# edwardyang12/Dex-NERF

Measured on AMD Instinct MI355X. Metric: rays/sec (64+128 samples) + PSNR vs ref, 400x400 scene, higher is better.
Workload: dtype bf16; 1 GPU; C2 render: 400x400 rays/step/GPU, 64 coarse + 128 fine samples, coarse+fine FlexibleNeRFModel D8/W256/skip4 + viewdirs, PE L=10/4, 20 Dex thresholds, validation mode (det. resampling, no noise)

## Files before the change

dex-nerf_amd/csrc/api.cpp:

```cpp
#include <cmath>
#include <cstdlib>
#include <cstring>
#include <utility>
#include <vector>

#include "../../include/dexnerf_hip_ext.h"
#include "../../include/dexnerf_hip_normals.h"
#include "../../include/dexnerf_hip_quantile.h"
#include "dn_common.h"
#include "composite_body.h"
#include "dn_rng.h"
#include "mlp_layout.h"

namespace dn {

static thread_local char g_err[512] = "";

void set_error(const char* fmt, ...) {
  va_list ap;
  va_start(ap, fmt);
  vsnprintf(g_err, sizeof(g_err), fmt, ap);
  va_end(ap);
}

// ... 18 lines not shown
    int cus = 256;
    if (hipDeviceGetAttribute(&cus, hipDeviceAttributeMultiprocessorCount, dev) != hipSuccess || cus <= 0) cus = 256;
    cache[dev] = cus;
  }
  return cache[dev];
}

static size_t align256(size_t v) { return (v + 255) & ~static_cast<size_t>(255); }

struct Workspace {
  float *z_c, *rf_c, *w_c, *z_f, *rf_f, *g_rf;
  unsigned* absmax_part;
  unsigned* status;
  size_t bytes;
};

static Workspace carve(void* base, int64_t n, int nc, int nf, bool train = false) {
  Workspace w{};
  size_t off = 0;
  auto take = [&](size_t floats) {
    float* p = base ? reinterpret_cast<float*>(static_cast<char*>(base) + off) : nullptr;
    off += align256(floats * sizeof(float));
    return p;
  };
  w.z_c = take(static_cast<size_t>(n) * nc);
  w.rf_c = take(static_cast<size_t>(n) * nc * 4);
  w.w_c = take(static_cast<size_t>(n) * nc);
  if (nf > 0) {
    w.z_f = take(static_cast<size_t>(n) * (nc + nf));
    w.rf_f = take(static_cast<size_t>(n) * (nc + nf) * 4);
// ... 85 lines not shown
  if ((rc = dn_coarse_depths(rays, ray_stride, n_rays, num_coarse, lindisp, t_rand, w.z_c, stream))) return rc;
  const bool fine = num_fine > 0;
  DN_REQUIRE(n_thres >= 0 && n_thres <= kMaxThres, "dn_render_rays: at most %d Dex thresholds", kMaxThres);
  auto comp_for = [&](float* rgb, float* acc, float* weights, float* depth, float* dex, int k) {
    CompParams c{};
    c.rgb = rgb; c.acc = acc; c.weights = weights; c.depth = depth; c.dex = dex; c.disp = nullptr;
    c.nonfinite = w.status; c.n_rays = n_rays; c.n_thres = k; c.white = white_background;
    for (int i = 0; i < kMaxThres; ++i) c.th.m[i] = (i < k) ? h_m_thres[i] : 0.0f;
    return c;
  };
  const bool may_fuse = !(noise_std > 0.0f);
  int done = 0;
  {
    const CompParams c = comp_for(rgb_c, acc_c, w.w_c, depth_c, fine ? nullptr : dex_f, fine ? 0 : n_thres);
    if ((rc = run_network_flagged(desc_coarse, precision, packed_coarse, nullptr, nullptr, rays, ray_stride, w.z_c, n_rays,
                                  num_coarse, w.rf_c, w.status + 1, stream, (may_fuse && rgb_c) ? &c : nullptr, &done)))
      return rc;
  }
  if (!done && (rc = volume_render_counting(w.rf_c, w.z_c, rays + 3, ray_stride, noise_c, noise_std, white_background, h_m_thres,
                                            fine ? 0 : n_thres, n_rays, num_coarse, rgb_c, nullptr, acc_c, w.w_c, depth_c,
                                            fine ? nullptr : dex_f, w.status, stream)))
    return rc;
  if (!fine) return 0;
  if ((rc = dn_fine_depths(w.z_c, w.w_c, u, n_rays, num_coarse, num_fine, w.z_f, nullptr, stream))) return rc;
  {
    const CompParams c = comp_for(rgb_f, acc_f, nullptr, depth_f, dex_f, n_thres);
    if ((rc = run_network_flagged(desc_fine, precision, packed_fine, nullptr, nullptr, rays, ray_stride, w.z_f, n_rays,
                                  num_coarse + num_fine, w.rf_f, w.status + 1, stream, (may_fuse && rgb_f) ? &c : nullptr, &done)))
      return rc;
  }
  if (done) return 0;
  return volume_render_counting(w.rf_f, w.z_f, rays + 3, ray_stride, noise_f, noise_std, white_background, h_m_thres, n_thres,
                                n_rays, num_coarse + num_fine, rgb_f, nullptr, acc_f, nullptr, depth_f, dex_f, w.status, stream);
}

extern "C" size_t dn_render_depth_workspace_bytes(int64_t n_rays, int num_coarse, int num_fine) {
  if (n_rays < 0 || num_coarse < 1 || num_fine < 0) return 0;
  return carve_depth(nullptr, n_rays, num_coarse, num_fine).bytes;
}

static int render_rays_depth_impl(const char* who, const dn_mlp_desc* desc_coarse, const void* packed_coarse, const dn_mlp_desc* desc_fine,
                                  const void* packed_fine, int precision, const float* rays, int ray_stride, int64_t n_rays,
                                  int num_coarse, int num_fine, int lindisp, float noise_std, const float* d_m_thres, int n_thres,
// ... 488 lines not shown
```

dex-nerf_amd/csrc/dn_common.h:

```cpp
#pragma once
#include <hip/hip_runtime.h>
#include <cstdarg>
#include <cstdint>
#include <cstdio>

#include "../../include/dexnerf_hip.h"

namespace dn {

constexpr int kWave = 64;

void set_error(const char* fmt, ...);

inline hipStream_t as_stream(dn_stream_t s) { return reinterpret_cast<hipStream_t>(s); }

inline int check_launch(const char* what) {
  hipError_t e = hipGetLastError();
  if (e != hipSuccess) {
    set_error("%s: %s", what, hipGetErrorString(e));
    return -static_cast<int>(e);
  }
  return 0;
}

// ... 18 lines not shown
                                int n_samples, float* depth, float* acc, float* dex, float* qdepth, unsigned* nonfinite,
                                dn_stream_t stream);

int composite_normals_counting(const float* rf, const float* z, const float* rd, int rd_stride, const float* noise, float noise_std,
                               const float* g_pts, const float* d_m_thres, int n_thres, int64_t n_rays, int n_samples, float* depth,
                               float* acc, float* dex, float* normal, float* dex_normal, unsigned* nonfinite, dn_stream_t stream);
int density_seed(float* g_out, int64_t n_points, dn_stream_t stream);
int input_grad_check(const dn_mlp_desc* desc, int precision, const char* who);
int input_grad_points_from_rays(const dn_mlp_desc* desc, int precision, const void* packed_ig, const void* grads, const float* rays,
                                int ray_stride, const float* z_vals, int64_t n_rays, int samples_per_ray, float* d_pts, dn_stream_t stream);

bool weight_grad_pair_fits(const dn_mlp_desc& d);
struct CompParams;
int run_network_flagged(const dn_mlp_desc* desc, int precision, const void* packed, const float* pts, const float* viewdirs,
                        const float* rays, int ray_stride, const float* z_vals, int64_t n_rays, int samples_per_ray, float* out,
                        unsigned* range_flag, dn_stream_t stream, const CompParams* comp = nullptr, int* composited = nullptr);

int coarse_depths_rng(const float* rays, int ray_stride, int64_t n_rays, int num_coarse, int lindisp, const float* t_rand,
                      float* z_vals, const uint32_t* rng_state, dn_stream_t stream);
int fine_depths_rng(const float* z_coarse, const float* weights, const float* u, int64_t n_rays, int num_coarse, int num_fine,
                    float* z_fine, float* z_samples, const uint32_t* rng_state, dn_stream_t stream);
int volume_render_backward_rng(const char* name, const float* rf, const float* z, const float* rd, int rd_stride, const float* noise,
                               float noise_std, int white_background, int64_t n_rays, int n_samples, const float* g_rgb,
                               const float* g_depth, const float* g_acc, const float* g_disp, const float* g_weights, float* g_rf,
                               float* g_z, float* g_rd, const uint32_t* rng_state, uint32_t rng_stream, unsigned* absmax_part,
                               dn_stream_t stream);
int coarse_depths_backward_rng(const float* rays, int ray_stride, int64_t n_rays, int num_coarse, int lindisp, const float* t_rand,
                               const float* g_z, const float* g_z_b, const float* g_z_c, float* g_near_far, const uint32_t* rng_state,
                               dn_stream_t stream);
int fine_depths_backward_sum(const float* z_coarse, const float* z_samples, const float* g_z_fine, const float* g_z_fine_b, int64_t n_rays,
                             int num_coarse, int num_fine, float* g_z_coarse, dn_stream_t stream);
// ... 123 lines not shown
```

dex-nerf_amd/csrc/mlp_fused.hip:

```cpp
#include "mlp_fused_kernel.h"
#include "mlp_internal.h"
#include "mlp_geo48.h"

namespace dn {

DN_FWD32_INSTANCES(DN_FWD32_EXTERN)


template <int BF16, int DENS = 0>
__global__ void pack_kernel(NetLayout L, PackPtrs ptrs, char* __restrict__ packed) {
  using P = Prec<BF16>;
  const int n_bias = L.total_bias_tiles * 32;
  float* bias_out = reinterpret_cast<float*>(packed);
  for (int idx = blockIdx.x * blockDim.x + threadIdx.x; idx < L.bias_bytes / 4; idx += gridDim.x * blockDim.x) {
    float v = 0.0f;
    if (idx < n_bias) {
      const int tile = idx / 32, hh = (idx % 32) / 16, r = idx % 16, s = pack_stage_of_bias_tile(L, tile);
      int src;
      const int n = pack_src_row<32>(L.st[s], tile - L.st[s].bias0, acc_row(r, hh), DENS && s == L.n_stages - 1, &src);
      if (n >= 0) v = ptrs.b[src][n];
    }
    bias_out[idx] = v;
  }
  char* wout = packed + L.bias_bytes;
// ... 51 lines not shown

template <int W, int LX, int LD, int BF16, int PT, int SAVE>
static int launch_forward(FwdParams p, hipStream_t stream) {
  auto kern = mlp_forward_kernel<W, LX, LD, BF16, PT, SAVE>;
  constexpr int WAVES = waves_of<BF16, PT>();
  constexpr int PTS_PER_WG = WAVES * 32 * PT;
  constexpr int KXP = kXyzPanel / (2 * Prec<BF16>::EPP);
  p.n_tiles = (p.n_points + PTS_PER_WG - 1) / PTS_PER_WG;
  constexpr int KDP = round_up(3 + 6 * LD, 16) / (2 * Prec<BF16>::EPP);
  const size_t lds = kRingBytes + p.bias_bytes + WAVES * (kInRows * 32 * PT * sizeof(float) + PT * (KXP + KDP) * kPieceBytes);
  if (int rc = ensure_big_lds(reinterpret_cast<const void*>(kern))) return rc;
  hipLaunchKernelGGL(kern, dim3(static_cast<unsigned>(persistent_grid(p.n_tiles))), dim3(WAVES * 64), lds, stream, p);
  return check_launch("mlp_forward");
}

int dispatch_forward(const dn_mlp_desc& d, int precision, FwdParams& p, hipStream_t stream, const CompParams* comp, int* composited) {
  const bool bf = precision == DN_PREC_BF16;
  const bool hf = precision == DN_PREC_F16;
  const char* region48 = p.packed + core_stream_bytes(p.bias_bytes, p.total_pieces);
  if ((bf || hf) && !read_switches().geom32 && p.act == nullptr && p.mode != 2 && p.n_points < (1LL << 31) - 1024 && g48_supported(d, precision))
    return launch_forward48(d, precision, p, region48, stream, comp, composited);
  if (p.act != nullptr && hf) { set_error("mlp_forward(train): fp16 is a render-only mode"); return DN_E_UNSUPPORTED; }
  if (p.act != nullptr && p.save8) {
    if (!bf || p.mode == 2 || !g48_train_supported(d) || p.n_points >= (1LL << 31) - 1024) {
      set_error("mlp_forward(train, 8-bit saved tensors): bf16 arithmetic, rays / points input, W in {128, 256}, L_xyz in {6, 10}, a depth the 48-point kernel holds in LDS");
      return DN_E_UNSUPPORTED;
    }
    return launch_forward48(d, precision, p, region48, stream);
  }
  const int prec_arg = bf ? 1 : hf ? 2 : 0;
  const int save = p.act != nullptr ? 1 : 0;
#define DN_CASE(W_, LX_, F_, SAVE_)                                                            \
  if (d.hidden_size == W_ && d.num_encoding_fn_xyz == LX_ && prec_arg == F_ && save == SAVE_) \
    return launch_forward<W_, LX_, 4, F_, 1, SAVE_>(p, stream);
  DN_FWD32_INSTANCES(DN_CASE)
#undef DN_CASE
// ... 108 lines not shown
  if (rc == 0 && g48_supported(d, precision))
    rc = launch_pack48(d, precision, ptrs, static_cast<char*>(packed) + core_stream_bytes(L.bias_bytes, L.total_pieces), as_stream(stream), true);
  return rc;
}

extern "C" int dn_run_network(const dn_mlp_desc* desc, int precision, const void* packed, const float* pts,
                              const float* viewdirs, const float* rays, int ray_stride, const float* z_vals,
                              int64_t n_rays, int samples_per_ray, float* out, dn_stream_t stream) {
  return dn::run_network_flagged(desc, precision, packed, pts, viewdirs, rays, ray_stride, z_vals, n_rays, samples_per_ray, out,
                                 nullptr, stream);
}

int dn::run_network_flagged(const dn_mlp_desc* desc, int precision, const void* packed, const float* pts,
                            const float* viewdirs, const float* rays, int ray_stride, const float* z_vals,
                            int64_t n_rays, int samples_per_ray, float* out, unsigned* range_flag, dn_stream_t stream,
                            const CompParams* comp, int* composited) {
  if (composited) *composited = 0;
  FwdParams p;
  int rc = setup_params(desc, precision, packed, &p);
  if (rc) return rc;
  if (n_rays == 0) return 0;
  DN_REQUIRE(packed && out && n_rays >= 0 && samples_per_ray >= 1, "dn_run_network: bad arguments");
  DN_REQUIRE((reinterpret_cast<uintptr_t>(out) & 15) == 0, "dn_run_network: out must be 16-byte aligned");
  if ((rc = set_point_inputs("dn_run_network", *desc, pts, viewdirs, rays, ray_stride, z_vals, n_rays, samples_per_ray, &p))) return rc;
  p.out = out;
  p.range_flag = range_flag;
  if (p.n_points == 0) return 0;
  return dispatch_forward(*desc, precision, p, as_stream(stream), comp, composited);
}

extern "C" int dn_mlp_forward_encoded(const dn_mlp_desc* desc, int precision, const void* packed, const float* x,
                                      int64_t n_rows, float* out, dn_stream_t stream) {
  FwdParams p;
  int rc = setup_params(desc, precision, packed, &p);
  if (rc) return rc;
  if (n_rows == 0) return 0;
  DN_REQUIRE(packed && x && out && n_rows >= 0, "dn_mlp_forward_encoded: bad arguments");
  DN_REQUIRE((reinterpret_cast<uintptr_t>(out) & 15) == 0, "dn_mlp_forward_encoded: out must be 16-byte aligned");
  p.mode = 2; p.enc = x;
  p.enc_ld = (3 + 6 * desc->num_encoding_fn_xyz) + (desc->use_viewdirs ? 3 + 6 * desc->num_encoding_fn_dir : 0);
  p.n_points = n_rows; p.S = 1; p.out = out;
  if (n_rows == 0) return 0;
  return dispatch_forward(*desc, precision, p, as_stream(stream));
// ... 2 lines not shown
```

dex-nerf_amd/csrc/mlp_fused48.hip:

```cpp
#include "mlp_fused48_kernel.h"

namespace dn {

DN_FWD48_INSTANCES(DN_FWD48_EXTERN)
template <int W, int F, int DC, unsigned MASKC, int VIEWC, int SAVE, int OVLP, int COMP>
__global__ __launch_bounds__(kG48Waves * 64, 2) void mlp_forward_density48_kernel(FwdParams p, G48Params q);
#define DN_FWD48_DENSITY_EXTERN(W, F, DC, MASKC, VIEWC, SAVE, OVLP, COMP) \
  extern template __global__ void mlp_forward_density48_kernel<W, F, DC, MASKC, VIEWC, SAVE, OVLP, COMP>(FwdParams, G48Params);
DN_FWD48_DENSITY(DN_FWD48_DENSITY_EXTERN)

template <int F, int DENS = 0>
__device__ __forceinline__ void pack48_body(const NetLayout& L, const PackPtrs& ptrs, const G48Tables& tabs, char* __restrict__ region);

template <int F, int DENS = 0>
__global__ void pack48_kernel(NetLayout L, PackPtrs ptrs, G48Tables tabs, char* __restrict__ region) {
  pack48_body<F, DENS>(L, ptrs, tabs, region);
}

template <int F>
__global__ void pack48_pair_kernel(NetLayout L, PackPtrs ptrs_a, PackPtrs ptrs_b, G48Tables tabs, char* __restrict__ region_a,
                                   char* __restrict__ region_b) {
  if (blockIdx.y == 0) pack48_body<F>(L, ptrs_a, tabs, region_a);
  else pack48_body<F>(L, ptrs_b, tabs, region_b);
}
// ... 74 lines not shown
  const G48Tables tabs = g48_tables(d);
  const dim3 blocks(pack48_blocks(L), b ? 2 : 1);
  if (b) {
    static_assert(sizeof(NetLayout) + 2 * sizeof(PackPtrs) + sizeof(G48Tables) + 16 <= 4096, "kernel arguments of the pair pack");
    hipLaunchKernelGGL(pack48_pair_kernel<1>, blocks, dim3(256), 0, stream, L, a, *b, tabs, region_a, region_b);
    return check_launch("mlp_pack48_pair");
  }
  with_prec<false>(precision, [&](auto f) {
    constexpr int F = decltype(f)::value;
    auto kern = density ? pack48_kernel<F, 1> : pack48_kernel<F, 0>;
    hipLaunchKernelGGL(kern, blocks, dim3(256), 0, stream, L, a, tabs, region_a);
  });
  return check_launch(density ? "mlp_pack48_density" : "mlp_pack48");
}

int launch_forward48(const dn_mlp_desc& d, int precision, const FwdParams& p_in, const char* region, hipStream_t stream,
                     const CompParams* comp, int* composited) {
  if (composited) *composited = 0;
  NetLayout L;
  build_layout48(d, &L);
  FwdParams p = p_in;
  G48Params q{};
  q.base = region; q.bias_bytes = L.bias_bytes; q.total_pieces = L.total_pieces;
  size_t lds = g48_lds_bytes(L);
  if (lds > 160 * 1024) { set_error("mlp_forward48: %zu bytes of LDS", lds); return DN_E_UNSUPPORTED; }
  const int cus = device_cus();
  const G48Pick pick = g48_pick(d, precision, p, comp, cus, read_switches());
  if (pick.refusal) { set_error("%s", pick.refusal); return DN_E_UNSUPPORTED; }
  const G48Key& k = pick.key;
  const int tile_points = k.SAVE == 3 ? 256 : kG48PointsPerWg;
  p.n_tiles = (p.n_points + tile_points - 1) / tile_points;
  if (k.OVLP == 1) lds += static_cast<size_t>(kG48Waves) * 3 * kG48PointsPerWave * sizeof(float);
  if (k.COMP) {
    q.comp = *comp;
    if (composited) *composited = 1;
  }
  auto launch = [&](auto kern) -> int {
    if (int rc = ensure_big_lds(reinterpret_cast<const void*>(kern))) return rc;
    hipLaunchKernelGGL(kern, dim3(static_cast<unsigned>(persistent_grid(p.n_tiles, cus))), dim3(kG48Waves * 64), lds, stream, p, q);
    return check_launch("mlp_forward48");
  };
#define DN_CASE(KERNEL, W, F, DC, MASKC, VIEWC, SAVE, OVLP, COMP) \
  if (k == G48Key{W, F, DC, MASKC, VIEWC, SAVE, OVLP, COMP}) return launch(KERNEL<W, F, DC, MASKC, VIEWC, SAVE, OVLP, COMP>);
#define DN_CASE_FWD(...) DN_CASE(mlp_forward48_kernel, __VA_ARGS__)
#define DN_CASE_DENSITY(...) DN_CASE(mlp_forward_density48_kernel, __VA_ARGS__)
  if (pick.density) { DN_FWD48_DENSITY(DN_CASE_DENSITY) }
  else { DN_FWD48_INSTANCES(DN_CASE_FWD) }
#undef DN_CASE_DENSITY
#undef DN_CASE_FWD
#undef DN_CASE
  set_error("mlp_forward48: the picked instance is not in the list");
  return DN_E_UNSUPPORTED;
}
// ... 3 lines not shown
```

dex-nerf_amd/csrc/mlp_fused48_kernel.h:

```cpp
#pragma once
#include "mlp_stage48.h"

namespace dn {


template <bool MAY_BE_IDENTITY = true>
__device__ __forceinline__ float pe_value(float xc, f32x4 entry) {
  const float rev = __builtin_amdgcn_fractf(xc * entry[0]) + entry[1];
  const float s = __builtin_amdgcn_sinf(rev);
  if constexpr (MAY_BE_IDENTITY) return entry[2] * xc + entry[3] * s;
  else return s;
}

__device__ __forceinline__ void rotate3(const float (&x)[3], int g, float (&xr)[3]) {
  const unsigned r = static_cast<unsigned>(g) % 3u;
  const unsigned m1 = 0u - (r & 1u), m2 = 0u - (r >> 1);
  const unsigned b0 = __float_as_uint(x[0]), b1 = __float_as_uint(x[1]), b2 = __float_as_uint(x[2]);
  xr[0] = __uint_as_float(b0 ^ ((b0 ^ b1) & m1) ^ ((b0 ^ b2) & m2));
  xr[1] = __uint_as_float(b1 ^ ((b1 ^ b2) & m1) ^ ((b1 ^ b0) & m2));
  xr[2] = __uint_as_float(b2 ^ ((b2 ^ b0) & m1) ^ ((b2 ^ b1) & m2));
}

template <int W, int F, int DC = 0, unsigned MASKC = 0, int VIEWC = 0, int SAVE = 0, int OVLP = 0, int COMP = 0>
__global__ __launch_bounds__(kG48Waves * 64, 2) void mlp_forward48_kernel(FwdParams p, G48Params q) {
// ... 59 lines not shown
      for (int c = 0; c < 3; ++c) dma(p.pts + static_cast<long long>(pt) * 3 + c, c);
      if (p.use_viewdirs) {
        const float* v = p.viewdirs + static_cast<long long>(pt / p.S) * 3;
#pragma unroll
        for (int c = 0; c < 3; ++c) dma(v + c, 7 + 3 * vset + c);
      }
    }
  };

  {
    const f32x4* gsrc = reinterpret_cast<const f32x4*>(q.base);
    f32x4* l = reinterpret_cast<f32x4*>(bias_lds);
    for (int i = threadIdx.x; i < (q.bias_bytes + kG48TableBytes) / 16; i += WAVES * 64) l[i] = gsrc[i];
  }
  issue_inputs(blockIdx.x, 0);
  const unsigned inbuf_addr = static_cast<unsigned>(reinterpret_cast<uintptr_t>((__attribute__((address_space(3))) char*)inbuf));
  auto issue_inputs_flat = [&](int tile, int set) {
    const int ln = fresh_lane();
    int pt = tile * PPG + wave * PPW + ln;
    pt = pt < n_points ? pt : n_points - 1;
    const float* r = p.rays + static_cast<long long>(pt / p.S) * p.ray_stride;
#pragma unroll
    for (int c = 0; c < 6; ++c) dma4_lanes48(r + c, inbuf_addr + c * (PPW * 4));
    dma4_lanes48(p.z + pt, inbuf_addr + 6 * (PPW * 4));
#pragma unroll
    for (int c = 0; c < 3; ++c) dma4_lanes48(r + 8 + c, inbuf_addr + (7 + c) * (PPW * 4) + set * (3 * PPW * 4));
  };

  Pipe48<WAVES> pipe;
  pipe.ring = ring;
// ... 34 lines not shown
    const f32x4* tabx = reinterpret_cast<const f32x4*>(tab_lds) + (lane >> 4) * 16;
#pragma unroll
    for (int u = 0; u < 16; ++u) {
      const f32x4 e = tabx[u];
      tfreq[u] = e[0]; tphase[u] = e[1];
      if (u < 3) { tw_id[u] = e[2]; tw_sin[u] = e[3]; }
    }
  }
  unsigned long long idm[3] = {0ull, 0ull, 0ull};
  if constexpr (OVX) {
    const f32x4* tabx = reinterpret_cast<const f32x4*>(tab_lds) + (lane >> 4) * 16;
#pragma unroll
    for (int u = 0; u < 3; ++u) idm[u] = __ballot(tabx[u][2] != 0.0f);
  }
  const int n_tiles = static_cast<int>(p.n_tiles);
  auto tile_loop = [&](auto role_c) __attribute__((always_inline)) {
  constexpr int ROLE = decltype(role_c)::value;
  if constexpr (SPLIT) first_reads();
  for (int tile = blockIdx.x; tile < n_tiles; tile += gridDim.x, vset = (VSETS == 2 ? vset ^ 1 : (vset == 2 ? 0 : vset + 1))) {
    const char* act_grp[PT] = {};
    const char* mask_base = nullptr;
    if constexpr (SAVE != 0) {
      const long long wt = static_cast<long long>(tile) * WAVES + wave;
#pragma unroll
      for (int t = 0; t < PT; ++t) {
        const long long G = wt * PT + t;
        act_grp[t] = uniform_ptr(p.act + ((G >> 1) * p.act_pieces * 2 + (G & 1)) * kPieceBytes);
      }
      mask_base = uniform_ptr(p.masks + wt * p.mask_words * (2 * kPieceBytes));
    }
    const bool first_tile = tile == static_cast<int>(blockIdx.x);
    if ((!OVL && !OVX) || first_tile) {
      const int ln = fresh_lane();
      const int j = ln & 15;
      const f32x4* tabx = reinterpret_cast<const f32x4*>(tab_lds) + (ln >> 4) * 16;
      char* pex = pex_of(ln);
      if (wave >= 4) asm volatile("s_waitcnt vmcnt(0)" ::: "memory");
      float in[PT][7];
#pragma unroll
      for (int t = 0; t < PT; ++t)
#pragma unroll
        for (int c = 0; c < 7; ++c) in[t][c] = inbuf[c * PPW + t * 16 + j];
      asm volatile("s_waitcnt lgkmcnt(0)" ::: "memory");
      {
        const int nxt = tile + gridDim.x;
        if (nxt < n_tiles) issue_inputs(nxt, vset ^ 1);
      }
#pragma unroll
      for (int t = 0; t < PT; ++t) {
        float x[3];
#pragma unroll
        for (int c = 0; c < 3; ++c)
          x[c] = (p.mode == 0) ? in[t][c] + in[t][3 + c] * in[t][6] : in[t][c];
        float xr[3];
        rotate3(x, ln >> 4, xr);
        BP8 pk[KXP];
#pragma unroll
        for (int k = 0; k < KXP; ++k) {
          BP8 piece;
#pragma unroll
// ... 146 lines not shown
        static_assert(SPLIT, "in-stage encoding: an instance whose pass is compiled per role");
        if constexpr (ROLE == kXsConsumer) asm volatile("s_waitcnt vmcnt(0)" ::: "memory");
        else asm volatile("" ::: "memory");
        const int ln = fresh_lane();
        const int j = ln & 15;
#pragma unroll
        for (int t = 0; t < PT; ++t)
#pragma unroll
          for (int c = 0; c < 7; ++c) in_n[t][c] = inbuf[c * PPW + t * 16 + j];
        tab_addr_v = pipe.ring_addr + kRingBytes + static_cast<unsigned>(q.bias_bytes) + static_cast<unsigned>(ln >> 4) * 256u;
        stash_addr_v = pipe.ring_addr + kRingBytes + static_cast<unsigned>(q.bias_bytes) + kG48TableBytes + wave * (PT * KXP * kPieceBytes) + static_cast<unsigned>(ln) * 16u;
        asm volatile("ds_read_b64 %0, %1" : "=v"(tbl[0]) : "v"(tab_addr_v));
      }
#pragma unroll
      for (int t = 0; t < PT; ++t) ped[t] = *reinterpret_cast<const BP8*>(pex_of(pipe.lane16 >> 4) + t * kPieceBytes);
      asm volatile("s_waitcnt lgkmcnt(0)" : "+v"(ped[0]), "+v"(ped[1]), "+v"(ped[2]), "+v"(pipe.af[0]), "+v"(pipe.af[1]), "+v"(pipe.bias_nxt), "+v"(tbl[0]));
      if constexpr (OVX) {
        const int t2 = tile + 2 * static_cast<int>(gridDim.x);
        issue_inputs_flat(t2 < n_tiles ? t2 : tile, vset);
        const int ln = fresh_lane();
#pragma unroll
        for (int t = 0; t < PT; ++t) {
          float x[3];
#pragma unroll
          for (int c = 0; c < 3; ++c) x[c] = in_n[t][c] + in_n[t][3 + c] * in_n[t][6];
          rotate3(x, ln >> 4, xr_n[t]);
        }
      }
      auto enc_hook = [&](auto b_c, auto w_c) {
        if constexpr (OVX) {
          constexpr int b = decltype(b_c)::value, w = decltype(w_c)::value;
          constexpr int q0 = enc_begin(b, KT_D), cap = enc_cap(b, KT_D);
          auto one = [&](auto q_c) {
            constexpr int qq = decltype(q_c)::value;
// ... 237 lines not shown
      for (; i + 1 < p.D - 1; i += 2) {
        trunk_layer(i, ba, bb);
        trunk_layer(i + 1, bb, ba);
      }
      if (i < p.D - 1) {
        trunk_layer(i, ba, bb);
#pragma unroll
        for (int t = 0; t < PT; ++t)
#pragma unroll
          for (int k = 0; k < KH; ++k) ba[t][k] = bb[t][k];
      }
      if (p.use_viewdirs) heads(ba, bb, std::true_type{});
      else heads(ba, bb, std::false_type{});
    }
    }
    const int lo = fresh_lane();
    if constexpr (COMP != 0) {
      f32x4* stage = reinterpret_cast<f32x4*>(smem + kRingBytes + q.bias_bytes + kG48TableBytes);
#pragma unroll
      for (int t = 0; t < PT; ++t) {
        if (lo < 16) {
          f32x4 o;
          o[0] = out4[t][0]; o[1] = out4[t][1]; o[2] = out4[t][2]; o[3] = out4[t][3];
          stage[wave * PPW + t * 16 + lo] = o;
        }
      }
      asm volatile("s_waitcnt lgkmcnt(0)" ::: "memory");
      __builtin_amdgcn_s_barrier();
      const int S = p.S;
      const int rays_per_tile = PPG / S;
// ... 9 lines not shown
      asm volatile("s_waitcnt lgkmcnt(0)" ::: "memory");
      __builtin_amdgcn_s_barrier();
    } else {
#pragma unroll
      for (int t = 0; t < PT; ++t) {
        const int pt = tile * PPG + wave * PPW + t * 16 + (lo & 15);
        if (pt < n_points && lo < 16) {
          f32x4 o;
          o[0] = out4[t][0]; o[1] = out4[t][1]; o[2] = out4[t][2]; o[3] = out4[t][3];
          __builtin_nontemporal_store(o, reinterpret_cast<f32x4*>(p.out + static_cast<long long>(pt) * 4));
        }
      }
    }
  }
  };
  if constexpr (SPLIT) {
    if (wave < 4) tile_loop(std::integral_constant<int, kXsFetcher>{});
    else tile_loop(std::integral_constant<int, kXsConsumer>{});
  } else {
    tile_loop(std::integral_constant<int, kXsFetcher>{});
  }
  asm volatile("s_waitcnt vmcnt(0) lgkmcnt(0)" ::: "memory");
  if constexpr (F == 2) {
    const bool out_of_range = (trk & 0xFFFFu) >= 0x7C00u || (trk >> 16) >= 0x7C00u;
    if (p.range_flag != nullptr && __ballot(out_of_range) != 0ull && (threadIdx.x & 63) == 0) atomicAdd(p.range_flag, 1u);
  }
}

#define DN_FWD48_PAPER_BF16_ENC(X) X(256, 1, 8, 0x10u, 1, 0, 2, 0)
#define DN_FWD48_PAPER_BF16_PLAIN(X) X(256, 1, 8, 0x10u, 1, 0, 0, 0)
#define DN_FWD48_PAPER_FP16_ENC(X) X(256, 2, 8, 0x10u, 1, 0, 2, 0)
#define DN_FWD48_PAPER_FP16_PLAIN(X) X(256, 2, 8, 0x10u, 1, 0, 0, 0)
#define DN_FWD48_PAPER_BF16(X) DN_FWD48_PAPER_BF16_ENC(X) DN_FWD48_PAPER_BF16_PLAIN(X)
#define DN_FWD48_PAPER_FP16(X) DN_FWD48_PAPER_FP16_ENC(X) DN_FWD48_PAPER_FP16_PLAIN(X)
#define DN_FWD48_W128(X)  \
  X(128, 1, 0, 0u, 0, 0, 0, 0) X(128, 2, 0, 0u, 0, 0, 0, 0)  \
  X(128, 1, 4, 0u, 1, 0, 0, 0) X(128, 2, 4, 0u, 1, 0, 0, 0)  \
// ... 20 lines not shown
```

dex-nerf_amd/csrc/mlp_geo48.h:

```cpp
#pragma once
#include "mlp_internal.h"
#include "composite_body.h"

namespace dn {

constexpr int kG48Waves = 8;
constexpr int kG48PointsPerWave = 48;
constexpr int kG48PointsPerWg = kG48Waves * kG48PointsPerWave;
constexpr int kG48XyzPieces = kXyzPanel / 32;
constexpr int kG48DirPieces = 1;
constexpr int kG48TableBytes = 1536;
constexpr int kG48InRows = 13;

__host__ __device__ inline int g48_pe_col(int kind, int g, int u, int L) {
  const int slots = kind == 1 ? 16 : 8;
  const int comp = (u + g) % 3;
  int rank = 0;
  for (int gg = 0; gg <= g; ++gg)
    for (int uu = 0; uu < (gg == g ? u : slots); ++uu) rank += ((uu + gg) % 3 == comp) ? 1 : 0;
  if (rank == 0) return comp;
  const int f = (rank - 1) / 2, is_cos = (rank - 1) % 2;
  return f < L ? 3 + 6 * f + 3 * is_cos + comp : -1;
}

__host__ __device__ constexpr int g48_hidden_col(int k, int g, int e) { return (2 * k + e / 4) * 16 + 4 * g + (e % 4); }

struct G48Tables {
  float fx[16];
  float fd[8];
  int LX, LD;
};

struct G48Params {
  const char* base;
  int bias_bytes;
  int total_pieces;
  CompParams comp;
};


inline int build_layout48(const dn_mlp_desc& d, NetLayout* out) {
  const int W = d.hidden_size, D = d.num_layers;
  const int DX = 3 + 6 * d.num_encoding_fn_xyz, DD = 3 + 6 * d.num_encoding_fn_dir;
  NetLayout& L = *out;
  L = NetLayout{};
  L.W = W; L.LX = d.num_encoding_fn_xyz; L.LD = d.num_encoding_fn_dir; L.D = D; L.use_viewdirs = d.use_viewdirs;
  int piece = 0, bias = 0, s = 0;
  auto add = [&](int n_tiles, int hidden_in, int pe_kind, int src, int src2, int n_real, int ld, int col_h0, int col_p0) {
    StageDesc& t = L.st[s++];
    t = StageDesc{};
    t.n_tiles = n_tiles; t.hidden_in = hidden_in; t.pe_kind = pe_kind; t.src = src; t.src2 = src2;
    t.n_real = n_real; t.ld = ld; t.col_hidden0 = col_h0; t.col_pe0 = col_p0;
    t.first_tile2 = (src2 >= 0) ? 0 : -1;
// ... 16 lines not shown
    add(1, W / 2, 0, i_rgb, -1, 3, W / 2, 0, 0);
  } else {
    add(1, W, 0, D, -1, 4, W, 0, 0);
  }
  L.n_stages = s;
  L.total_pieces = round_up(piece, kPhasePieces);
  L.total_bias_tiles = bias;
  L.bias_bytes = round_up(bias * 64, 1024);
  return 0;
}

inline size_t g48_lds_bytes(const NetLayout& L) {
  return static_cast<size_t>(kRingBytes) + L.bias_bytes + kG48TableBytes + kG48Waves * 3 * kG48XyzPieces * kPieceBytes +
         kG48Waves * kG48InRows * kG48PointsPerWave * sizeof(float);
}

inline bool g48_supported(const dn_mlp_desc& d, int precision) {
  if ((precision != DN_PREC_BF16 && precision != DN_PREC_F16) || (d.hidden_size != 256 && d.hidden_size != 128)) return false;
  NetLayout L;
  build_layout48(d, &L);
  return g48_lds_bytes(L) <= 160 * 1024;
}

inline unsigned pack48_blocks(const NetLayout& L) {
  const long long elems = static_cast<long long>(L.total_pieces) * 512;
  const long long b = (elems + 511) / 512;
  return static_cast<unsigned>(b < 64 ? 64 : (b > 4096 ? 4096 : b));
}

inline size_t g48_region_bytes(const dn_mlp_desc& d) {
// ... 159 lines not shown
  if (p.act != nullptr) {
    if (precision != DN_PREC_BF16 || !p.save8)
      return G48Pick{G48Key{}, false, "mlp_forward48(train): the 48-point training forward is the bf16 / 8-bit-saved-tensor mode"};
    if (sh.two_group(sw) && g48_train_groups(p.n_points, cus, sw) == 2) return fixed(3, 0, 0);
    return (paper || shipped) ? fixed(2, 0, 0) : run_time(2);
  }
  if (sh.density_fixed() && !sw.runtime_shape)
    return G48Pick{sh.paper_trunk ? G48Key{256, F, 8, 0x10u, 0, 0, 0, 0} : G48Key{128, F, 4, 0u, 0, 0, 0, 0}, true, nullptr};
  if (comp != nullptr && comp->rgb != nullptr && (paper || shipped) && p.mode == 0 && p.S >= 1 && kG48PointsPerWg % p.S == 0 &&
      comp->n_rays * p.S == p.n_points && sw.fused_composite)
    return fixed(0, 0, 1);
  if ((paper || shipped) && p.mode == 0 && !sw.no_overlap) return fixed(0, shipped ? 1 : 2, 0);
  return (paper || shipped) ? fixed(0, 0, 0) : run_time(0);
}

int launch_pack48(const dn_mlp_desc& d, int precision, const PackPtrs& a, char* region_a, hipStream_t stream, bool density = false,
                  const PackPtrs* b = nullptr, char* region_b = nullptr);
int launch_forward48(const dn_mlp_desc& d, int precision, const FwdParams& p, const char* region, hipStream_t stream,
                     const CompParams* comp = nullptr, int* composited = nullptr);
int backward48_entry(const dn_mlp_desc* desc, const void* packed_bwd, const float* g_out, const void* masks, int64_t n_points,
                     void* grads, float grad_scale, hipStream_t stream, const unsigned* partials = nullptr, int n_partials = 0);
int unpack48_entry(const dn_mlp_desc* desc, int which, const void* native, int64_t n_points, int slot, int width, int kind, float* out,
                   int ld_out, int col0, hipStream_t stream);
int launch_pack48_backward(const dn_mlp_desc& d, const PackPtrs& a, char* packed_a, hipStream_t stream, const PackPtrs* b = nullptr,
                           char* packed_b = nullptr);

}
```

dex-nerf_amd/csrc/mlp_internal.h:

```cpp
#pragma once
#include "mlp_device.h"
#include <type_traits>

namespace dn {

struct PackPtrs {
  const float* w[kMaxStages];
  const float* b[kMaxStages];
};

__device__ __forceinline__ int pack_stage_of_piece(const NetLayout& L, int piece) {
  int s = 0;
  while (s + 1 < L.n_stages && L.st[s + 1].piece0 <= piece) ++s;
  return s;
}
__device__ __forceinline__ int pack_stage_of_bias_tile(const NetLayout& L, int tile) {
  int s = 0;
  while (s + 1 < L.n_stages && L.st[s + 1].bias0 <= tile) ++s;
  return s;
}
template <int ROWS>
__device__ __forceinline__ int pack_src_row(const StageDesc& st, int ts, int i, bool dens_head, int* src) {
  *src = st.src;
  if (st.src2 >= 0) {
// ... 50 lines not shown
}
template <class Layout>
inline void copy_act_slots(const Layout& t, FwdParams* p) {
  p->slot_xyz = t.slot_xyz; p->slot_dir = t.slot_dir; p->slot_layer1 = t.slot_layer1; p->slot_trunk0 = t.slot_trunk0;
  p->slot_feat = t.slot_feat; p->slot_dirout = t.slot_dirout;
}
template <class Layout, class Params>
inline void copy_grad_slots(const Layout& t, Params* p) {
  p->gslot_dirout = t.gslot_dirout; p->gslot_feat = t.gslot_feat; p->gslot_trunk0 = t.gslot_trunk0; p->gslot_layer1 = t.gslot_layer1;
  p->gslot_out = t.gslot_out;
}
inline long long persistent_grid(long long n_tiles, int cus = device_cus()) { return n_tiles < cus ? n_tiles : cus; }

int setup_params(const dn_mlp_desc* desc, int precision, const void* packed, FwdParams* p);
struct CompParams;
int dispatch_forward(const dn_mlp_desc& d, int precision, FwdParams& p, hipStream_t stream, const CompParams* comp = nullptr, int* composited = nullptr);
int launch_pack(const NetLayout& L, const PackPtrs& ptrs, void* packed, int precision, hipStream_t stream, bool density = false);
void fill_freqs(float* f, int num_fns, int log_sampling);

}
```

Baseline: 5.467 million rays/s.

## Use atomic dynamic tile claiming in persistent fused MLP kernel

```diff
diff --git a/dex-nerf_amd/csrc/api.cpp b/dex-nerf_amd/csrc/api.cpp
--- a/dex-nerf_amd/csrc/api.cpp
+++ b/dex-nerf_amd/csrc/api.cpp
@@ -56,6 +56,7 @@
   unsigned* status;
   size_t bytes;
 };
+constexpr int kStatusTilesCoarse = 16, kStatusTilesFine = 32;
 
 static Workspace carve(void* base, int64_t n, int nc, int nf, bool train = false) {
   Workspace w{};
@@ -171,7 +172,8 @@
   {
     const CompParams c = comp_for(rgb_c, acc_c, w.w_c, depth_c, fine ? nullptr : dex_f, fine ? 0 : n_thres);
     if ((rc = run_network_flagged(desc_coarse, precision, packed_coarse, nullptr, nullptr, rays, ray_stride, w.z_c, n_rays,
-                                  num_coarse, w.rf_c, w.status + 1, stream, (may_fuse && rgb_c) ? &c : nullptr, &done)))
+                                  num_coarse, w.rf_c, w.status + 1, stream, (may_fuse && rgb_c) ? &c : nullptr, &done,
+                                  w.status + kStatusTilesCoarse)))
       return rc;
   }
   if (!done && (rc = volume_render_counting(w.rf_c, w.z_c, rays + 3, ray_stride, noise_c, noise_std, white_background, h_m_thres,
@@ -183,7 +185,8 @@
   {
     const CompParams c = comp_for(rgb_f, acc_f, nullptr, depth_f, dex_f, n_thres);
     if ((rc = run_network_flagged(desc_fine, precision, packed_fine, nullptr, nullptr, rays, ray_stride, w.z_f, n_rays,
-                                  num_coarse + num_fine, w.rf_f, w.status + 1, stream, (may_fuse && rgb_f) ? &c : nullptr, &done)))
+                                  num_coarse + num_fine, w.rf_f, w.status + 1, stream, (may_fuse && rgb_f) ? &c : nullptr, &done,
+                                  w.status + kStatusTilesFine)))
       return rc;
   }
   if (done) return 0;
diff --git a/dex-nerf_amd/csrc/dn_common.h b/dex-nerf_amd/csrc/dn_common.h
--- a/dex-nerf_amd/csrc/dn_common.h
+++ b/dex-nerf_amd/csrc/dn_common.h
@@ -56,7 +56,8 @@
 struct CompParams;
 int run_network_flagged(const dn_mlp_desc* desc, int precision, const void* packed, const float* pts, const float* viewdirs,
                         const float* rays, int ray_stride, const float* z_vals, int64_t n_rays, int samples_per_ray, float* out,
-                        unsigned* range_flag, dn_stream_t stream, const CompParams* comp = nullptr, int* composited = nullptr);
+                        unsigned* range_flag, dn_stream_t stream, const CompParams* comp = nullptr, int* composited = nullptr,
+                        unsigned* tile_counter = nullptr);
 
 int coarse_depths_rng(const float* rays, int ray_stride, int64_t n_rays, int num_coarse, int lindisp, const float* t_rand,
                       float* z_vals, const uint32_t* rng_state, dn_stream_t stream);
diff --git a/dex-nerf_amd/csrc/mlp_fused.hip b/dex-nerf_amd/csrc/mlp_fused.hip
--- a/dex-nerf_amd/csrc/mlp_fused.hip
+++ b/dex-nerf_amd/csrc/mlp_fused.hip
@@ -89,12 +89,13 @@
   return check_launch("mlp_forward");
 }
 
-int dispatch_forward(const dn_mlp_desc& d, int precision, FwdParams& p, hipStream_t stream, const CompParams* comp, int* composited) {
+int dispatch_forward(const dn_mlp_desc& d, int precision, FwdParams& p, hipStream_t stream, const CompParams* comp, int* composited,
+                     unsigned* tile_counter) {
   const bool bf = precision == DN_PREC_BF16;
   const bool hf = precision == DN_PREC_F16;
   const char* region48 = p.packed + core_stream_bytes(p.bias_bytes, p.total_pieces);
   if ((bf || hf) && !read_switches().geom32 && p.act == nullptr && p.mode != 2 && p.n_points < (1LL << 31) - 1024 && g48_supported(d, precision))
-    return launch_forward48(d, precision, p, region48, stream, comp, composited);
+    return launch_forward48(d, precision, p, region48, stream, comp, composited, tile_counter);
   if (p.act != nullptr && hf) { set_error("mlp_forward(train): fp16 is a render-only mode"); return DN_E_UNSUPPORTED; }
   if (p.act != nullptr && p.save8) {
     if (!bf || p.mode == 2 || !g48_train_supported(d) || p.n_points >= (1LL << 31) - 1024) {
@@ -233,7 +234,7 @@
 int dn::run_network_flagged(const dn_mlp_desc* desc, int precision, const void* packed, const float* pts,
                             const float* viewdirs, const float* rays, int ray_stride, const float* z_vals,
                             int64_t n_rays, int samples_per_ray, float* out, unsigned* range_flag, dn_stream_t stream,
-                            const CompParams* comp, int* composited) {
+                            const CompParams* comp, int* composited, unsigned* tile_counter) {
   if (composited) *composited = 0;
   FwdParams p;
   int rc = setup_params(desc, precision, packed, &p);
@@ -245,7 +246,7 @@
   p.out = out;
   p.range_flag = range_flag;
   if (p.n_points == 0) return 0;
-  return dispatch_forward(*desc, precision, p, as_stream(stream), comp, composited);
+  return dispatch_forward(*desc, precision, p, as_stream(stream), comp, composited, tile_counter);
 }
 
 extern "C" int dn_mlp_forward_encoded(const dn_mlp_desc* desc, int precision, const void* packed, const float* x,
diff --git a/dex-nerf_amd/csrc/mlp_fused48.hip b/dex-nerf_amd/csrc/mlp_fused48.hip
--- a/dex-nerf_amd/csrc/mlp_fused48.hip
+++ b/dex-nerf_amd/csrc/mlp_fused48.hip
@@ -112,8 +112,31 @@
   return check_launch(density ? "mlp_pack48_density" : "mlp_pack48");
 }
 
+#ifdef DN_TILE_STAMP
+static unsigned long long* g_tile_stamps = nullptr;
+static long long g_tile_stamp_launches = 0;
+constexpr size_t kTileStampLaunchWords = static_cast<size_t>(kTileStampMaxWgs) * kTileStampWords;
+static unsigned long long* tile_stamp_slot(long long grid) {
+  if (grid > kTileStampMaxWgs) return nullptr;
+  if (g_tile_stamps == nullptr) {
+    const size_t bytes = kTileStampLaunches * kTileStampLaunchWords * sizeof(unsigned long long);
+    if (hipMalloc(reinterpret_cast<void**>(&g_tile_stamps), bytes) != hipSuccess) { g_tile_stamps = nullptr; return nullptr; }
+    if (hipMemset(g_tile_stamps, 0, bytes) != hipSuccess) return nullptr;
+  }
+  return g_tile_stamps + static_cast<size_t>(g_tile_stamp_launches++ % kTileStampLaunches) * kTileStampLaunchWords;
+}
+}
+extern "C" __attribute__((visibility("default"))) long long dn_tile_stamp_read(unsigned long long* dst) {
+  using namespace dn;
+  if (g_tile_stamps == nullptr || hipDeviceSynchronize() != hipSuccess) return -1;
+  if (hipMemcpy(dst, g_tile_stamps, kTileStampLaunches * kTileStampLaunchWords * sizeof(unsigned long long), hipMemcpyDeviceToHost) != hipSuccess) return -1;
+  return g_tile_stamp_launches;
+}
+namespace dn {
+#endif
+
 int launch_forward48(const dn_mlp_desc& d, int precision, const FwdParams& p_in, const char* region, hipStream_t stream,
-                     const CompParams* comp, int* composited) {
+                     const CompParams* comp, int* composited, unsigned* tile_counter) {
   if (composited) *composited = 0;
   NetLayout L;
   build_layout48(d, &L);
@@ -129,12 +152,19 @@
   const int tile_points = k.SAVE == 3 ? 256 : kG48PointsPerWg;
   p.n_tiles = (p.n_points + tile_points - 1) / tile_points;
   if (k.OVLP == 1) lds += static_cast<size_t>(kG48Waves) * 3 * kG48PointsPerWave * sizeof(float);
+  if (g48_claims(k) && lds + kG48ClaimBytes <= 160 * 1024) {
+    lds += kG48ClaimBytes;
+    q.tile_counter = tile_counter;
+  }
   if (k.COMP) {
     q.comp = *comp;
     if (composited) *composited = 1;
   }
   auto launch = [&](auto kern) -> int {
     if (int rc = ensure_big_lds(reinterpret_cast<const void*>(kern))) return rc;
+#ifdef DN_TILE_STAMP
+    q.stamp = tile_stamp_slot(persistent_grid(p.n_tiles, cus));
+#endif
     hipLaunchKernelGGL(kern, dim3(static_cast<unsigned>(persistent_grid(p.n_tiles, cus))), dim3(kG48Waves * 64), lds, stream, p, q);
     return check_launch("mlp_forward48");
   };
diff --git a/dex-nerf_amd/csrc/mlp_fused48_kernel.h b/dex-nerf_amd/csrc/mlp_fused48_kernel.h
--- a/dex-nerf_amd/csrc/mlp_fused48_kernel.h
+++ b/dex-nerf_amd/csrc/mlp_fused48_kernel.h
@@ -97,6 +97,17 @@
     for (int i = threadIdx.x; i < (q.bias_bytes + kG48TableBytes) / 16; i += WAVES * 64) l[i] = gsrc[i];
   }
   issue_inputs(blockIdx.x, 0);
+  constexpr bool CLAIM = XS && W == 256 && OVLP == 2;
+  unsigned* const claim_lds = reinterpret_cast<unsigned*>(smem + kRingBytes + q.bias_bytes + kG48TableBytes + WAVES * PT * KXP * kPieceBytes +
+                                                          WAVES * IN_ROWS * PPW * sizeof(float));
+  const bool claim = CLAIM && q.tile_counter != nullptr;
+  if constexpr (CLAIM) {
+    if (claim && threadIdx.x == 4 * 64) {
+      const unsigned v = gridDim.x + __hip_atomic_fetch_add(q.tile_counter, 2u, __ATOMIC_RELAXED, __HIP_MEMORY_SCOPE_AGENT);
+      claim_lds[0] = v;
+      claim_lds[1] = v + 1u;
+    }
+  }
   const unsigned inbuf_addr = static_cast<unsigned>(reinterpret_cast<uintptr_t>((__attribute__((address_space(3))) char*)inbuf));
   auto issue_inputs_flat = [&](int tile, int set) {
     const int ln = fresh_lane();
@@ -161,10 +172,22 @@
     for (int u = 0; u < 3; ++u) idm[u] = __ballot(tabx[u][2] != 0.0f);
   }
   const int n_tiles = static_cast<int>(p.n_tiles);
+  int next_tile = static_cast<int>(blockIdx.x + gridDim.x), after_next = 0;
+  if constexpr (CLAIM) {
+    if (claim) next_tile = __builtin_amdgcn_readfirstlane(static_cast<int>(claim_lds[0]));
+  }
+  unsigned claimed = 0u;
+  auto advance = [&](int tile) {
+    if constexpr (CLAIM) { const int t = next_tile; next_tile = after_next; return t; }
+    else return tile + static_cast<int>(gridDim.x);
+  };
+#ifdef DN_TILE_STAMP
+  int tiles_run = 0;
+#endif
   auto tile_loop = [&](auto role_c) __attribute__((always_inline)) {
   constexpr int ROLE = decltype(role_c)::value;
   if constexpr (SPLIT) first_reads();
-  for (int tile = blockIdx.x; tile < n_tiles; tile += gridDim.x, vset = (VSETS == 2 ? vset ^ 1 : (vset == 2 ? 0 : vset + 1))) {
+  for (int tile = blockIdx.x; tile < n_tiles; tile = advance(tile), vset = (VSETS == 2 ? vset ^ 1 : (vset == 2 ? 0 : vset + 1))) {
     const char* act_grp[PT] = {};
     const char* mask_base = nullptr;
     if constexpr (SAVE != 0) {
@@ -177,6 +200,9 @@
       mask_base = uniform_ptr(p.masks + wt * p.mask_words * (2 * kPieceBytes));
     }
     const bool first_tile = tile == static_cast<int>(blockIdx.x);
+#ifdef DN_TILE_STAMP
+    ++tiles_run;
+#endif
     if ((!OVL && !OVX) || first_tile) {
       const int ln = fresh_lane();
       const int j = ln & 15;
@@ -190,7 +216,7 @@
         for (int c = 0; c < 7; ++c) in[t][c] = inbuf[c * PPW + t * 16 + j];
       asm volatile("s_waitcnt lgkmcnt(0)" ::: "memory");
       {
-        const int nxt = tile + gridDim.x;
+        const int nxt = CLAIM ? next_tile : tile + static_cast<int>(gridDim.x);
         if (nxt < n_tiles) issue_inputs(nxt, vset ^ 1);
       }
 #pragma unroll
@@ -367,10 +393,35 @@
       }
 #pragma unroll
       for (int t = 0; t < PT; ++t) ped[t] = *reinterpret_cast<const BP8*>(pex_of(pipe.lane16 >> 4) + t * kPieceBytes);
-      asm volatile("s_waitcnt lgkmcnt(0)" : "+v"(ped[0]), "+v"(ped[1]), "+v"(ped[2]), "+v"(pipe.af[0]), "+v"(pipe.af[1]), "+v"(pipe.bias_nxt), "+v"(tbl[0]));
+      unsigned claim_q = 0u;
+      if constexpr (CLAIM) {
+        claim_q = claim_lds[1];
+        asm volatile("s_waitcnt lgkmcnt(0)" : "+v"(ped[0]), "+v"(ped[1]), "+v"(ped[2]), "+v"(pipe.af[0]), "+v"(pipe.af[1]), "+v"(pipe.bias_nxt), "+v"(tbl[0]), "+v"(claim_q));
+      } else {
+        asm volatile("s_waitcnt lgkmcnt(0)" : "+v"(ped[0]), "+v"(ped[1]), "+v"(ped[2]), "+v"(pipe.af[0]), "+v"(pipe.af[1]), "+v"(pipe.bias_nxt), "+v"(tbl[0]));
+      }
       if constexpr (OVX) {
-        const int t2 = tile + 2 * static_cast<int>(gridDim.x);
+        int t2 = tile + 2 * static_cast<int>(gridDim.x);
+        if constexpr (CLAIM) {
+          if (claim) t2 = __builtin_amdgcn_readfirstlane(static_cast<int>(claim_q));
+          after_next = t2;
+        }
         issue_inputs_flat(t2 < n_tiles ? t2 : tile, vset);
+        if constexpr (CLAIM && ROLE == kXsConsumer) {
+          const unsigned m = __builtin_amdgcn_readfirstlane((claim && wave == 4 && next_tile < n_tiles) ? 1u : 0u);
+          const unsigned* ctr = q.tile_counter;
+          const unsigned one = 1u;
+          unsigned c = claimed;
+          asm volatile(
+              "s_mov_b32 exec_lo, %[m]\n\t"
+              "s_mov_b32 exec_hi, 0\n\t"
+              "global_atomic_add %[r], %[a], %[o], off sc0\n\t"
+              "s_mov_b64 exec, -1"
+              : [r] "+v"(c)
+              : [m] "s"(m), [a] "v"(ctr), [o] "v"(one)
+              : "memory");
+          claimed = c;
+        }
         const int ln = fresh_lane();
 #pragma unroll
         for (int t = 0; t < PT; ++t) {
@@ -638,6 +689,21 @@
       else heads(ba, bb, std::false_type{});
     }
     }
+    if constexpr (CLAIM && ROLE == kXsConsumer) {
+      unsigned c = claimed;
+      asm volatile("s_waitcnt vmcnt(0)" : "+v"(c) : : "memory");
+      const unsigned id = c + gridDim.x;
+      const unsigned m = __builtin_amdgcn_readfirstlane((claim && wave == 4) ? 1u : 0u);
+      const unsigned word1 = pipe.ring_addr + static_cast<unsigned>(reinterpret_cast<char*>(claim_lds) - smem) + 4u;
+      asm volatile(
+          "s_mov_b32 exec_lo, %[m]\n\t"
+          "s_mov_b32 exec_hi, 0\n\t"
+          "ds_write_b32 %[a], %[v]\n\t"
+          "s_mov_b64 exec, -1"
+          :
+          : [m] "s"(m), [a] "v"(word1), [v] "v"(id)
+          : "memory");
+    }
     const int lo = fresh_lane();
     if constexpr (COMP != 0) {
       f32x4* stage = reinterpret_cast<f32x4*>(smem + kRingBytes + q.bias_bytes + kG48TableBytes);
@@ -677,6 +743,14 @@
     }
   }
   };
+#ifdef DN_TILE_STAMP
+  unsigned long long* const stamp_rec = q.stamp + static_cast<size_t>(blockIdx.x) * kTileStampWords;
+  const bool stamps = q.stamp != nullptr && wave == WAVES - 1;
+  if (stamps && lane == 0) {
+    stamp_rec[0] = __builtin_amdgcn_s_memrealtime();
+    stamp_rec[1] = __builtin_amdgcn_s_memtime();
+  }
+#endif
   if constexpr (SPLIT) {
     if (wave < 4) tile_loop(std::integral_constant<int, kXsFetcher>{});
     else tile_loop(std::integral_constant<int, kXsConsumer>{});
@@ -684,6 +758,18 @@
     tile_loop(std::integral_constant<int, kXsFetcher>{});
   }
   asm volatile("s_waitcnt vmcnt(0) lgkmcnt(0)" ::: "memory");
+#ifdef DN_TILE_STAMP
+  if (stamps && lane == 0) {
+    unsigned xcc;
+    asm volatile("s_getreg_b32 %0, hwreg(HW_REG_XCC_ID, 0, 4)" : "=s"(xcc));
+    stamp_rec[2] = __builtin_amdgcn_s_memrealtime();
+    stamp_rec[3] = __builtin_amdgcn_s_memtime();
+    stamp_rec[4] = xcc;
+    stamp_rec[5] = static_cast<unsigned>(tiles_run);
+    stamp_rec[6] = gridDim.x;
+    stamp_rec[7] = static_cast<unsigned>(n_tiles);
+  }
+#endif
   if constexpr (F == 2) {
     const bool out_of_range = (trk & 0xFFFFu) >= 0x7C00u || (trk >> 16) >= 0x7C00u;
     if (p.range_flag != nullptr && __ballot(out_of_range) != 0ull && (threadIdx.x & 63) == 0) atomicAdd(p.range_flag, 1u);
diff --git a/dex-nerf_amd/csrc/mlp_geo48.h b/dex-nerf_amd/csrc/mlp_geo48.h
--- a/dex-nerf_amd/csrc/mlp_geo48.h
+++ b/dex-nerf_amd/csrc/mlp_geo48.h
@@ -36,7 +36,14 @@
   int bias_bytes;
   int total_pieces;
   CompParams comp;
-};
+  unsigned* tile_counter;
+#ifdef DN_TILE_STAMP
+  unsigned long long* stamp;
+#endif
+};
+constexpr int kTileStampWords = 8;
+constexpr int kTileStampMaxWgs = 1024;
+constexpr int kTileStampLaunches = 4;
 
 
 inline int build_layout48(const dn_mlp_desc& d, NetLayout* out) {
@@ -83,6 +90,8 @@
   return static_cast<size_t>(kRingBytes) + L.bias_bytes + kG48TableBytes + kG48Waves * 3 * kG48XyzPieces * kPieceBytes +
          kG48Waves * kG48InRows * kG48PointsPerWave * sizeof(float);
 }
+
+constexpr int kG48ClaimBytes = 16;
 
 inline bool g48_supported(const dn_mlp_desc& d, int precision) {
   if ((precision != DN_PREC_BF16 && precision != DN_PREC_F16) || (d.hidden_size != 256 && d.hidden_size != 128)) return false;
@@ -272,10 +281,12 @@
   return (paper || shipped) ? fixed(0, 0, 0) : run_time(0);
 }
 
+inline bool g48_claims(const G48Key& k) { return k.W == 256 && k.DC > 0 && k.VIEWC != 0 && k.SAVE == 0 && k.OVLP == 2 && k.COMP == 0; }
+
 int launch_pack48(const dn_mlp_desc& d, int precision, const PackPtrs& a, char* region_a, hipStream_t stream, bool density = false,
                   const PackPtrs* b = nullptr, char* region_b = nullptr);
 int launch_forward48(const dn_mlp_desc& d, int precision, const FwdParams& p, const char* region, hipStream_t stream,
-                     const CompParams* comp = nullptr, int* composited = nullptr);
+                     const CompParams* comp = nullptr, int* composited = nullptr, unsigned* tile_counter = nullptr);
 int backward48_entry(const dn_mlp_desc* desc, const void* packed_bwd, const float* g_out, const void* masks, int64_t n_points,
                      void* grads, float grad_scale, hipStream_t stream, const unsigned* partials = nullptr, int n_partials = 0);
 int unpack48_entry(const dn_mlp_desc* desc, int which, const void* native, int64_t n_points, int slot, int width, int kind, float* out,
diff --git a/dex-nerf_amd/csrc/mlp_internal.h b/dex-nerf_amd/csrc/mlp_internal.h
--- a/dex-nerf_amd/csrc/mlp_internal.h
+++ b/dex-nerf_amd/csrc/mlp_internal.h
@@ -88,7 +88,8 @@
 
 int setup_params(const dn_mlp_desc* desc, int precision, const void* packed, FwdParams* p);
 struct CompParams;
-int dispatch_forward(const dn_mlp_desc& d, int precision, FwdParams& p, hipStream_t stream, const CompParams* comp = nullptr, int* composited = nullptr);
+int dispatch_forward(const dn_mlp_desc& d, int precision, FwdParams& p, hipStream_t stream, const CompParams* comp = nullptr, int* composited = nullptr,
+                     unsigned* tile_counter = nullptr);
 int launch_pack(const NetLayout& L, const PackPtrs& ptrs, void* packed, int precision, hipStream_t stream, bool density = false);
 void fill_freqs(float* f, int num_fns, int log_sampling);
 
```

New measurement: 5.601 million rays/s, median of 6. 1.02x the previous value.
